# MaartenGr/PolyFuzz

Measured on AMD Instinct MI355X. Metric: string-pairs/sec, TF-IDF cosine top-n 100k x 100k (config.timed_step says what a step is: by default the user-level .match() call of SURVEY section 8d's metric, `device_step` = the list resident in HBM; latency.top1_single_query_ms = top-1 match latency), higher is better.
Workload: dtype f32

## Files before the change

include/polyfuzz_hip.h:

```cpp
#ifndef POLYFUZZ_HIP_H
#define POLYFUZZ_HIP_H

#include <stdint.h>

#ifdef __cplusplus
extern "C" {
#endif

#define PFZ_VERSION 100

typedef enum pfz_status {
    PFZ_OK = 0,
    PFZ_ERR_INVALID = -1,
    PFZ_ERR_NO_DEVICE = -2,
    PFZ_ERR_HIP = -3,
    PFZ_ERR_UNSUPPORTED = -4,
    PFZ_ERR_NOMEM = -5,
    PFZ_ERR_RCCL = -6
} pfz_status;

typedef struct pfz_ctx pfz_ctx;
typedef struct pfz_csr pfz_csr;
typedef struct pfz_index pfz_index;
typedef struct pfz_topn pfz_topn;
// ... 22 lines not shown

int pfz_csr_upload(pfz_ctx *ctx, int64_t n_rows, int64_t n_cols,
                   const int64_t *indptr, const int32_t *indices, const float *data,
                   pfz_csr **out);
int pfz_csr_shape(const pfz_csr *m, int64_t *n_rows, int64_t *n_cols, int64_t *nnz);
int pfz_csr_download(pfz_ctx *ctx, const pfz_csr *m, int64_t *indptr, int32_t *indices, float *data);
void pfz_csr_free(pfz_csr *m);

int pfz_index_build(pfz_ctx *ctx, const pfz_csr *to_matrix, pfz_index **out);
void pfz_index_free(pfz_index *ix);
int pfz_index_info(const pfz_index *ix, int64_t *n_rows, int64_t *n_cols, int64_t *nnz,
                   int64_t *block_cols, int64_t *n_blocks, int64_t *table_bytes);
int pfz_index_pieces(const pfz_index *ix, int64_t *n_pieces, int64_t *piece_postings);
int pfz_index_symmetric_launches(const pfz_index *ix, int64_t *launches, int64_t *rows);
int pfz_index_symmetric_census(const pfz_index *ix, int64_t *magnet_rows, int64_t *recomputed_rows);

int pfz_topn_alloc(pfz_ctx *ctx, int64_t n_rows, int32_t ntop, pfz_topn **out);
void pfz_topn_free(pfz_topn *t);
int pfz_topn_clear(pfz_ctx *ctx, pfz_topn *t);
int pfz_topn_download(pfz_ctx *ctx, const pfz_topn *t, int32_t *out_idx, float *out_val);
int pfz_topn_download_rows_after(pfz_ctx *ctx, const pfz_topn *t, int64_t row_begin, int64_t row_end,
                                 int32_t event_slot, int32_t *out_idx, float *out_val);
int pfz_topn_rows_begin(pfz_ctx *ctx, const pfz_topn *t, int64_t row_begin, int64_t row_end, int32_t event_slot, int32_t half);
int pfz_topn_rows_finish(pfz_ctx *ctx, int32_t half, const int32_t **idx, const float **val);
int pfz_topn_upload(pfz_ctx *ctx, pfz_topn *t, const int32_t *idx, const float *val);
int pfz_topn_device_ptrs(const pfz_topn *t, void **idx_dev, void **val_dev, int64_t *n_rows, int32_t *ntop);

int pfz_cossim_topn(pfz_ctx *ctx, const pfz_index *to_index, const pfz_csr *from_matrix,
                    int32_t ntop, float lower_bound, int32_t exclude_diag, int64_t diag_offset,
                    pfz_topn *out);
// ... 203 lines not shown
```

polyfuzz_amd/_lib.py:

```python
import ctypes
import os
import threading

import numpy as np

from . import _build

c_i32, c_i64, c_f32, c_f64 = ctypes.c_int32, ctypes.c_int64, ctypes.c_float, ctypes.c_double
c_vp = ctypes.c_void_p
P = ctypes.POINTER


class PfzError(RuntimeError):
    def __init__(self, code, msg):
        super().__init__(f"libpolyfuzz_hip error {code}: {msg}")
        self.code = code


class PfzUnsupported(PfzError, NotImplementedError):
    pass


class PfzNoDevice(PfzError):
    pass
# ... 16 lines not shown
    "pfz_event_record": (ctypes.c_int, [c_vp, c_i32]),
    "pfz_event_elapsed_ms": (ctypes.c_int, [c_vp, c_i32, c_i32, P(c_f32)]),
    "pfz_prof_enable": (ctypes.c_int, [c_vp, c_i32]),
    "pfz_prof_reset": (ctypes.c_int, [c_vp]),
    "pfz_prof_get": (ctypes.c_int, [c_vp, ctypes.c_char_p, P(c_f64), P(c_i64)]),
    "pfz_csr_upload": (ctypes.c_int, [c_vp, c_i64, c_i64, c_vp, c_vp, c_vp, P(c_vp)]),
    "pfz_csr_shape": (ctypes.c_int, [c_vp, P(c_i64), P(c_i64), P(c_i64)]),
    "pfz_csr_download": (ctypes.c_int, [c_vp, c_vp, c_vp, c_vp, c_vp]),
    "pfz_csr_free": (None, [c_vp]),
    "pfz_index_build": (ctypes.c_int, [c_vp, c_vp, P(c_vp)]),
    "pfz_index_free": (None, [c_vp]),
    "pfz_index_info": (ctypes.c_int, [c_vp, P(c_i64), P(c_i64), P(c_i64), P(c_i64), P(c_i64), P(c_i64)]),
    "pfz_index_pieces": (ctypes.c_int, [c_vp, P(c_i64), P(c_i64)]),
    "pfz_index_symmetric_launches": (ctypes.c_int, [c_vp, P(c_i64), P(c_i64)]),
    "pfz_index_symmetric_census": (ctypes.c_int, [c_vp, P(c_i64), P(c_i64)]),
    "pfz_index_symmetric_ok": (ctypes.c_int, [c_vp, c_vp, c_i32, c_i32, P(c_i32)]),
    "pfz_comm_cossim_topn_symmetric": (ctypes.c_int, [c_vp, c_vp, c_vp, c_i32, ctypes.c_float, c_vp]),
    "pfz_comm_symmetric_ok": (ctypes.c_int, [c_vp, c_vp, c_vp, c_i32, P(c_i32)]),
    "pfz_rccl_versions": (ctypes.c_int, [P(c_i32), P(c_i32)]),
    "pfz_topn_alloc": (ctypes.c_int, [c_vp, c_i64, c_i32, P(c_vp)]),
    "pfz_topn_free": (None, [c_vp]),
    "pfz_topn_download": (ctypes.c_int, [c_vp, c_vp, c_vp, c_vp]),
    "pfz_topn_clear": (ctypes.c_int, [c_vp, c_vp]),
    "pfz_topn_download_rows_after": (ctypes.c_int, [c_vp, c_vp, c_i64, c_i64, c_i32, c_vp, c_vp]),
    "pfz_topn_rows_begin": (ctypes.c_int, [c_vp, c_vp, c_i64, c_i64, c_i32, c_i32]),
    "pfz_topn_rows_finish": (ctypes.c_int, [c_vp, c_i32, P(c_vp), P(c_vp)]),
    "pfz_cossim_topn_ranges": (ctypes.c_int, [c_vp, c_vp, c_vp, c_i32, ctypes.c_float, c_i32, c_i32, P(c_i64), c_i32, c_vp, P(c_vp), P(c_vp)]),
    "pfz_event_wait": (ctypes.c_int, [c_vp, c_i32]),
    "pfz_stage_reserve": (ctypes.c_int, [c_vp, c_i64, P(c_vp)]),
    "pfz_topn_upload": (ctypes.c_int, [c_vp, c_vp, c_vp, c_vp]),
# ... 281 lines not shown
    def symmetric_launches(self):
        a, b = c_i64(), c_i64()
        check(self.ctx.lib.pfz_index_symmetric_launches(self.h, ctypes.byref(a), ctypes.byref(b)))
        return a.value, b.value

    def symmetric_ok(self, csr, ntop, n_parts=1):
        yes = c_i32()
        check(self.ctx.lib.pfz_index_symmetric_ok(self.h, csr.h, int(ntop), int(n_parts), ctypes.byref(yes)))
        return bool(yes.value)

    def symmetric_census(self):
        a, b = c_i64(), c_i64()
        check(self.ctx.lib.pfz_index_symmetric_census(self.h, ctypes.byref(a), ctypes.byref(b)))
        return a.value, b.value


class DeviceTopN(_Handle):
    _free = "pfz_topn_free"

    @classmethod
    def alloc(cls, ctx, n_rows, ntop):
        h = c_vp()
        check(ctx.lib.pfz_topn_alloc(ctx.h, int(n_rows), int(ntop), ctypes.byref(h)))
        t = cls(ctx, h)
        t.n_rows, t.ntop = int(n_rows), int(ntop)
        return t

    def download(self):
        idx = np.empty((self.n_rows, self.ntop), np.int32)
        val = np.empty((self.n_rows, self.ntop), np.float32)
# ... 1035 lines not shown
```

polyfuzz_amd/csrc/k3_symmetric.hip:

```cpp
#include "k3_core.h"

#include <stdio.h>
#include <stdlib.h>

namespace pfz {

constexpr int kSymC = 2048;
constexpr int kSymCap = 96;
constexpr int kSymKeep = 32;
#ifndef PFZ_K3_SYM_F
#define PFZ_K3_SYM_F 128
#endif
#ifndef PFZ_K3_SYM_PUSH
#define PFZ_K3_SYM_PUSH 512
#endif
constexpr int kSymF = PFZ_K3_SYM_F;
constexpr int kSymPush = PFZ_K3_SYM_PUSH;
constexpr int kSymMergeCap = kSymPush + 64;
#ifndef PFZ_K3_SYM_SIDE_STREAMS
#define PFZ_K3_SYM_SIDE_STREAMS 2
#endif
constexpr int kSymSides = PFZ_K3_SYM_SIDE_STREAMS;
static_assert(kSymSides >= 1 && kSymSides <= 4, "one to four side streams");
constexpr int kSymSlices = 8;
constexpr int kSymSlicedRows = 4096;
#ifndef PFZ_K3_SYM_EXP
#define PFZ_K3_SYM_EXP 0
#endif
constexpr int kSymMag = 1;
constexpr int kSymMagBlocks = 8;
constexpr int kSymP0PerCu = 128;
constexpr int kSymDoneStride = 32;
constexpr int kNoThr = 0x7fffffff;

struct K3SymArgs {
    const int32_t *a_indptr;
    const int32_t *a_idx;
    const float *a_val;
    int32_t n;
    const int32_t *tab;
    const int2 *post;
    const int2 *post_sym;
    const uint16_t *pblk;
    const int32_t *n_pieces1;
    int32_t nb, ntop, thr0;
    float scale, inv_scale;
    int32_t row_begin, row_end;
    int32_t n_parts, my_part, per;
    int32_t thr_by_part;
    uint64_t *keys_out;
    int32_t *thrv;
    uint16_t *slot4;
    uint32_t *gmin;
    int32_t *thr_slot;
    uint16_t *row_slot;
    int32_t *mag;
    int32_t n_mag_items, mag_b0, mag_row_end;
    uint64_t *keys;
    int32_t *push_cnt;
    uint64_t *push_buf;
    int32_t *ovf;
    uint64_t *part;
    int32_t ovf_base, ovf_max, n_sl;
    int32_t *out_idx;
    float *out_val;
    int32_t *host_idx;
    float *host_val;
    uint32_t *done;
    int32_t blk_lo, blk_hi;
};

// ... 1 lines not shown
{
    return a.thr_by_part ? (row % a.n_parts) * a.per + row / a.n_parts : row;
}
__device__ inline bool row_is_mine(const K3SymArgs &a, int row) { return a.n_parts == 1 || row % a.n_parts == a.my_part; }


__host__ __device__ inline int sym_slot(int rho, int i, int *t, int *l, int *e)
{
    const int p = i >> 1, half = i & 1, c = rho & 3;
    *t = p >> 3;
    *l = (rho >> 2) + 8 * (p & 7);
    *e = half * 4 + c;
    return 512 * *t + 256 * half + 4 * *l + c;
}

__global__ __launch_bounds__(1024) void k3_sym_order(const K3SymArgs a)
{
    __shared__ int s_gmin[256];
    const int b = blockIdx.x, lane = threadIdx.x & 63, wave = threadIdx.x >> 6;
    if (threadIdx.x < 256) s_gmin[threadIdx.x] = kNoThr;
    if (threadIdx.x == 0 && a.done) a.done[b * kSymDoneStride] = 0u;
    __syncthreads();
    for (int rho = wave * 2; rho < wave * 2 + 2; ++rho) {
        const int r = rho + 32 * lane;
        const int row = b * kSymC + r;
        if (row < a.n) a.push_cnt[row] = 0;
        const int thr = row < a.n ? a.thrv[thr_pos(a, row)] : kNoThr;
        const uint64_t key = ((uint64_t)(uint32_t)thr << 6) | (uint32_t)lane;
        int rank = 0;
#pragma unroll 16
        for (int m = 0; m < 64; ++m) {
            const uint32_t lo = (uint32_t)__builtin_amdgcn_readlane((int)(uint32_t)key, m);
            const uint32_t hi = (uint32_t)__builtin_amdgcn_readlane((int)(uint32_t)(key >> 32), m);
            rank += ((((uint64_t)hi << 32) | lo) < key) ? 1 : 0;
        }
        int t, l, e;
        const int slot = sym_slot(rho, rank, &t, &l, &e);
        const bool magnet = rank < kSymMag && row < a.n && b > 0;
        if (rank < kSymMag) a.mag[(int64_t)b * (32 * kSymMag) + rho * kSymMag + rank] = magnet ? row : -1;
        a.slot4[(int64_t)b * kSymC + r] = (uint16_t)(slot * 4);
        a.thr_slot[(int64_t)b * kSymC + slot] = magnet ? kNoThr : thr;
        a.row_slot[(int64_t)b * kSymC + slot] = (uint16_t)r;
        if (!magnet) atomicMin(&s_gmin[t * 64 + l], thr);
    }
    __syncthreads();
    if (threadIdx.x < 64) {
        uint32_t w = 0;
        for (int t = 0; t < 4; ++t) {
            const int g = s_gmin[t * 64 + threadIdx.x];
            w |= (g == kNoThr ? 0xffu : (uint32_t)g >> 24) << (8 * t);
        }
        a.gmin[(int64_t)b * 64 + threadIdx.x] = w;
    }
}

__global__ __launch_bounds__(256) void k3_sym_repost(const K3SymArgs a)
{
    const int64_t i = (int64_t)blockIdx.x * 256 + threadIdx.x;
    if (i >= (int64_t)*a.n_pieces1 * (kPiece / 2)) return;
    const int piece = (int)(i >> 3);
    const int b = a.pblk[piece];
    int4 e = ((const int4 *)a.post)[i];
    const uint16_t *s4 = a.slot4 + (int64_t)b * kSymC;
    if (piece > 0) {
        e.x = s4[e.x >> 2];
        e.z = s4[e.z >> 2];
    }
// ... 38 lines not shown
    }
    const uint64_t t0 = wall_clock64();
    for (int b0 = a.blk_lo; b0 < a.blk_hi; b0 += 64) {
        const int b = b0 + lane;
        const bool on = b < a.blk_hi;
        const uint32_t want = on ? sym_items_of_block(a, b) : 0u;
        for (;;) {
            const uint32_t got = on ? __hip_atomic_load(&a.done[b * kSymDoneStride], __ATOMIC_RELAXED, __HIP_MEMORY_SCOPE_AGENT) : 0u;
            if (!__ballot(got < want)) break;
            if (wall_clock64() - t0 > 1000000000ull) __builtin_trap();
            __builtin_amdgcn_s_sleep(32);
        }
    }
}

template <int kCap>
__device__ inline void drain_stage(uint64_t *cand, TopState &st, uint64_t *fbuf, int &fcnt, int ntop, int lane,
                                   const K3SymArgs &a, uint32_t inv_row)
{
    wave_sync();
    for (int e0 = 0; e0 < fcnt; e0 += 64) {
        const bool on = e0 + lane < fcnt;
        const uint64_t en = on ? fbuf[e0 + lane] : 0ull;
        const uint32_t lo = (uint32_t)en;
        const int cell = (int)(lo & 0x3fffffffu);
        const int x = (int)(uint32_t)(en >> 32);
        int rowl = 0, thr = kNoThr;
        if (on) {
            rowl = a.row_slot[cell];
            thr = a.thr_slot[cell];
        }
        const int row = (cell & ~(kSymC - 1)) + rowl;
#if PFZ_K3_SYM_EXP == 5
        if (false) {
#else
        if ((lo & kStageFgn) && x > thr) {
#endif
            const int pos = atomicAdd(&a.push_cnt[row], 1);
            if (pos < kSymPush) store_coherent(&a.push_buf[(int64_t)row * kSymPush + pos], (en & 0xffffffff00000000ull) | inv_row);
        }
        const bool own = (lo & kStageOwn) && x > st.thr;
        const uint64_t mo = __ballot(own);
        if (mo) {
            const int pos = st.cnt + __popcll(mo & ((1ull << lane) - 1ull));
            if (own) cand[pos] = (en & 0xffffffff00000000ull) | (uint32_t)(~row);
            st.cnt += __popcll(mo);
            st.pushed = 1;
            if (st.cnt > kCap - 64) compact<kCap>(cand, st, ntop, lane, false);
        }
    }
    wave_sync();
    fcnt = 0;
}

template <int kCap>
__device__ inline void stage1(uint64_t *cand, TopState &st, uint64_t *fbuf, int &fcnt, int x, uint32_t tgu, int cell, int ntop,
                              int lane, const K3SymArgs &a, uint32_t inv_row)
{
    const bool own = x > st.thr, fgn = (uint32_t)x >= tgu;
    const uint64_t mk = __ballot(own || fgn);
    if (mk) {
        const int pos = fcnt + __popcll(mk & ((1ull << lane) - 1ull));
        if (own || fgn)
            fbuf[pos] = ((uint64_t)(uint32_t)x << 32) | (own ? kStageOwn : 0u) | (fgn ? kStageFgn : 0u) | (uint32_t)cell;
        fcnt += __popcll(mk);
        if (fcnt > kSymF - 64) drain_stage<kCap>(cand, st, fbuf, fcnt, ntop, lane, a, inv_row);
    }
}

template <int kCap>
__device__ inline void stage8(uint64_t *cand, TopState &st, uint64_t *fbuf, int &fcnt, const int4 &v0, const int4 &v1, int pa,
                              int pb, int pc, uint32_t tgu, int cell0, int cell1, int ntop, int lane, const K3SymArgs &a,
                              uint32_t inv_row)
{
    if (__ballot(pa > st.thr || (uint32_t)pa >= tgu)) {
        stage1<kCap>(cand, st, fbuf, fcnt, v0.x, tgu, cell0, ntop, lane, a, inv_row);
        stage1<kCap>(cand, st, fbuf, fcnt, v0.y, tgu, cell0 + 1, ntop, lane, a, inv_row);
        stage1<kCap>(cand, st, fbuf, fcnt, v0.z, tgu, cell0 + 2, ntop, lane, a, inv_row);
    }
    if (__ballot(pb > st.thr || (uint32_t)pb >= tgu)) {
        stage1<kCap>(cand, st, fbuf, fcnt, v0.w, tgu, cell0 + 3, ntop, lane, a, inv_row);
        stage1<kCap>(cand, st, fbuf, fcnt, v1.x, tgu, cell1, ntop, lane, a, inv_row);
        stage1<kCap>(cand, st, fbuf, fcnt, v1.y, tgu, cell1 + 1, ntop, lane, a, inv_row);
    }
    if (__ballot(pc > st.thr || (uint32_t)pc >= tgu)) {
        stage1<kCap>(cand, st, fbuf, fcnt, v1.z, tgu, cell1 + 2, ntop, lane, a, inv_row);
        stage1<kCap>(cand, st, fbuf, fcnt, v1.w, tgu, cell1 + 3, ntop, lane, a, inv_row);
    }
}

template <int B> __device__ inline uint64_t top_byte_reaches(int mx, uint32_t q)
{
    uint64_t m;
    if (B == 0) asm("v_cmp_ge_u32_sdwa %0, %1, %2 src0_sel:BYTE_3 src1_sel:BYTE_0" : "=s"(m) : "v"(mx), "v"(q));
    else asm("v_cmp_ge_u32_sdwa %0, %1, %2 src0_sel:BYTE_3 src1_sel:BYTE_1" : "=s"(m) : "v"(mx), "v"(q));
    return m;
}

template <int N4, int kCap>
__device__ inline void sweep_block_handover(int4 *acc4, uint64_t *cand, TopState &st, int b, int ntop, int lane, int zero,
                                            uint32_t tq, uint64_t *fbuf, int &fcnt, const K3SymArgs &a, uint32_t inv_row)
{
    static_assert(N4 / 128 == 4, "four sweep steps per block");
#pragma unroll 1
    for (int h = 0; h < 2; ++h) {
#pragma unroll
        for (int u = 0; u < 2; ++u) {
            const int t = 2 * h + u;
            const int i0 = t * 128 + lane, i1 = i0 + 64;
            const int4 v0 = acc4[i0], v1 = acc4[i1];
            acc4[i0] = make_int4(zero, zero, zero, zero);
            acc4[i1] = make_int4(zero, zero, zero, zero);
            const int pa = max3i(v0.x, v0.y, v0.z), pb = max3i(v0.w, v1.x, v1.y), pc = max(v1.z, v1.w);
            const int mx = max3i(pa, pb, pc);
            const uint64_t hit = __ballot(mx > st.thr) | (u == 0 ? top_byte_reaches<0>(mx, tq) : top_byte_reaches<1>(mx, tq));
            if (hit)
                stage8<kCap>(cand, st, fbuf, fcnt, v0, v1, pa, pb, pc, (u == 0 ? tq << 24 : tq << 16) & 0xff000000u, b * kSymC + i0 * 4,
                             b * kSymC + i1 * 4, ntop, lane, a, inv_row);
        }
        tq >>= 16;
    }
}

__device__ inline void store_result(const K3SymArgs &a, int row, int r, uint64_t key)
{
    if (a.keys_out) {
        a.keys_out[(int64_t)row * a.ntop + r] = key;
    } else {
        const int32_t j = key ? (int32_t)(~(uint32_t)key) : -1;
        const float v = key ? (float)(int32_t)(uint32_t)(key >> 32) * a.inv_scale : 0.f;
        a.out_idx[(int64_t)row * a.ntop + r] = j;
        a.out_val[(int64_t)row * a.ntop + r] = v;
        if (a.host_idx) {
// ... 41 lines not shown
    const int n_sl = mode == 2 ? a.n_sl : 1;
    const int per_sl = (nb + n_sl - 1) / n_sl;
    if (mode == 2) {
        int n_ovf = a.ovf[0];
        n_ovf = n_ovf > a.n ? a.n : n_ovf;
        const int hi = n_ovf < a.ovf_base + a.ovf_max ? n_ovf : a.ovf_base + a.ovf_max;
        n_items = hi > a.ovf_base ? (hi - a.ovf_base) * n_sl : 0;
    }
    bool pf_ready = false;
    int pf_p0 = 0, pf_p1 = 0, pf_k = 0, pf_cur = 0, pf_nxt = 0;
    float pf_v = 0.f;
    for (int item = blockIdx.x; item < n_items; item += gridDim.x) {
        int row = mode == 2 ? a.ovf[1 + a.ovf_base + item / n_sl] : a.row_begin + item * a.n_parts;
        bool magnet = false;
        int m_lo = 0;
        if (mode == 1) {
            if (item < a.n_mag_items) {
                const int ns = (nb - 1 + kSymMagBlocks - 1) / kSymMagBlocks;
                const int mm = item / ns;
                m_lo = (item - mm * ns) * kSymMagBlocks;
                const int mblk = a.mag_b0 + mm / (32 * kSymMag);
                row = __builtin_amdgcn_readfirstlane(a.mag[(int64_t)mblk * (32 * kSymMag) + mm % (32 * kSymMag)]);
                if (row < a.row_begin || row >= a.mag_row_end || m_lo >= row / C || !row_is_mine(a, row)) {
                    sym_item_done(a, mblk, lane);
                    continue;
                }
                magnet = true;
            } else {
                row -= a.n_mag_items * a.n_parts;
                if (row >= (nb - 1) * C) continue;
            }
        }
        const int own = row / C;
        int b_lo = 0, b_hi = nb, b_first = own;
        if (mode == 2 && n_sl > 1) {
            b_lo = (item % n_sl) * per_sl;
            b_hi = b_lo + per_sl < nb ? b_lo + per_sl : nb;
            b_first = own >= b_lo && own < b_hi ? own : b_lo;
            if (b_lo >= b_hi) {
                if (lane < ntop) a.part[(int64_t)item * ntop + lane] = 0ull;
                continue;
            }
        }
        if (mode == 0) {
            b_lo = own;
// ... 11 lines not shown
            p0 = pf_p0;
            p1 = pf_p1;
        } else {
            p0 = a.a_indptr[row];
            p1 = a.a_indptr[row + 1];
        }
        const bool more = mode == 0 && item + (int)gridDim.x < n_items;
        const int row2 = a.row_begin + (item + (int)gridDim.x) * a.n_parts;
        int q0 = 0, q1 = 0;
        if (more) {
            q0 = a.a_indptr[row2];
            q1 = a.a_indptr[row2 + 1];
        }
        const int nnz = p1 - p0;
        const int self_col = mode == 1 ? -1 : row;
        const uint32_t inv_row = ~(uint32_t)row;
        TopState st;
        st.cnt = 0;
        st.thr = a.thr0;
        st.pushed = 0;
        bool warmed = false;
        if (mode == 1) {
            st.thr = a.thrv[thr_pos(a, row)];
            const uint64_t k = lane < ntop && !magnet ? a.keys[(int64_t)row * ntop + lane] : 0ull;
            st.cnt = __popcll(__ballot(k != 0ull));
            if (k) cand[lane] = k;
            warmed = true;
            wave_sync();
        }
        int fcnt = 0;

        const int n_blk = b_hi - b_lo;
        int cur0 = 0, nxt0 = 0;
        float as0 = 0.f;
        const bool have0 = lane < nnz;
        const int32_t *trow = a.tab;
        if (have0 && mode == 0 && pf_ready) {
            as0 = pf_v * a.scale;
            trow = a.tab + (int64_t)pf_k * nb;
            cur0 = pf_cur;
            nxt0 = pf_nxt;
        } else if (have0) {
            as0 = a.a_val[p0 + lane] * a.scale;
            trow = a.tab + (int64_t)a.a_idx[p0 + lane] * nb;
            cur0 = trow[b_first];
            nxt0 = trow[b_first + 1];
        }
        const bool have2 = more && lane < q1 - q0;

        uint32_t tq_next = 0xffffffffu;
#if PFZ_K3_SYM_EXP != 1
        if (mode == 1 && !magnet) tq_next = a.gmin[(int64_t)b_first * 64 + lane];
#endif
        for (int it = 0, b = b_first; it < n_blk; ++it) {
            const int s = cur0, e = have0 ? nxt0 : cur0;
            const int b_next = b + 1 < b_hi ? b + 1 : b_lo;
            const uint32_t tq = tq_next;
            bool touched = __ballot(e > s) != 0;
#if PFZ_K3_SYM_EXP == 13
            if (touched && mode != 0) scatter_pieces(acc, post_bytes, mark, e - s, s, as0, lane, src4, sub8, dummy_addr);
#else
// ... 24 lines not shown
                    scatter_pieces(acc, post_bytes, mark, e2 - s2, s2, as2, lane, src4, sub8, dummy_addr);
                }
            }
            if (touched) {
                wave_sync();
                if (!warmed) {
                    warmed = true;
#if PFZ_K3_SYM_EXP != 10
                    if (ntop <= kWarmMaxTop) {
                        const int t = warm_threshold<N4>(acc4, 0, ntop + 1, lane);
                        st.thr = t > st.thr ? t : st.thr;
                    }
#endif
                }
                if (mode == 1)
                    sweep_block_handover<N4, kSymCap>(acc4, cand, st, b, ntop, lane, zero, tq, fbuf, fcnt, a, inv_row);
#if PFZ_K3_SYM_EXP == 12
                else if (mode != 0)
#else
                else
#endif
                    sweep_block<N4, kSymCap>(acc4, cand, st, b * C, self_col, ntop, lane, zero);
                wave_sync();
            }
            if (mode == 0 && have2) {
                const int32_t *t2 = a.tab + (int64_t)pf_k * nb + row2 / C;
                pf_cur = t2[0];
                pf_nxt = t2[1];
            }
            b = b_next;
        }
        if (mode == 0) {
            pf_ready = more;
            pf_p0 = q0;
            pf_p1 = q1;
        }

        if (mode == 1 && fcnt) drain_stage<kSymCap>(cand, st, fbuf, fcnt, ntop, lane, a, inv_row);
#if PFZ_K3_SYM_EXP == 11
        if (mode != 0)
#endif
        compact<kSymCap>(cand, st, ntop, lane);
        if (mode == 1 && magnet) {
            if (lane < st.cnt) {
                const int pos = atomicAdd(&a.push_cnt[row], 1);
                if (pos < kSymPush) store_coherent(&a.push_buf[(int64_t)row * kSymPush + pos], cand[lane]);
            }
        } else if (mode == 2 && n_sl > 1) {
            if (lane < ntop) a.part[(int64_t)item * ntop + lane] = lane < st.cnt ? cand[lane] : 0ull;
        } else if (mode == 2) {
            for (int r = lane; r < ntop; r += 64) store_result(a, row, r, r < st.cnt ? cand[r] : 0ull);
        } else {
            if (lane < ntop) {
                const uint64_t k = lane < st.cnt ? cand[lane] : 0ull;
                if (mode == 1) store_coherent(&a.keys[(int64_t)row * ntop + lane], k);
                else a.keys[(int64_t)row * ntop + lane] = k;
            }
            if (mode == 0 && lane == 0) a.thrv[thr_pos(a, row)] = st.thr;
        }
        if (mode == 1) sym_item_done(a, own, lane);
        wave_sync();
// ... 64 lines not shown
            const uint64_t k = e0 + lane < total ? a.part[(int64_t)r * total + e0 + lane] : 0ull;
            const uint64_t mk = __ballot(k != 0ull);
            if (k) cand[st.cnt + __popcll(mk & ((1ull << lane) - 1ull))] = k;
            st.cnt += __popcll(mk);
        }
        compact<256>(cand, st, ntop, lane);
        for (int q = lane; q < ntop; q += 64) store_result(a, row, q, q < st.cnt ? cand[q] : 0ull);
        wave_sync();
    }
}


struct K3SymState {
    int64_t n = 0;
    DevBuf thrv, slot4, gmin, thr_slot, row_slot, mag, post_sym, keys, push_cnt, push_buf, ovf, part;
    DevBuf ovfx[3], partx[3];
    DevBuf done;
    int64_t next_row = -1;
    uint64_t a_serial = 0;
    const pfz_topn *out = nullptr;
    int32_t ntop = 0, thr0 = 0;
    float scale = 0.f;
    int64_t launches = 0, rows = 0;
};

void k3_sym_free(pfz_index *ix)
{
    delete ix->sym;
    ix->sym = nullptr;
}
// ... 16 lines not shown
    if (force == 1) return 1;
    if (ix->n_rows < knob_int(knob::K3_SYM_MIN, 20480) || ix->n_rows > 250000) return 0;
    return (row_end - row_begin) * 5 >= ix->n_rows ? 1 : 0;
}

static int sym_state_alloc(pfz_ctx *ctx, const pfz_index *ix, K3SymState *s)
{
    const int64_t n = ix->n_rows;
    const size_t cells = (size_t)ix->n_blocks * kSymC;
    PFZ_TRY(s->thrv.alloc(ctx, (size_t)(n + 64) * sizeof(int32_t)));
    PFZ_TRY(s->slot4.alloc(ctx, cells * sizeof(uint16_t)));
    PFZ_TRY(s->gmin.alloc(ctx, cells / 32 * sizeof(uint32_t)));
    PFZ_TRY(s->thr_slot.alloc(ctx, cells * sizeof(int32_t)));
    PFZ_TRY(s->row_slot.alloc(ctx, cells * sizeof(uint16_t)));
    PFZ_TRY(s->mag.alloc(ctx, (size_t)ix->n_blocks * 32 * kSymMag * sizeof(int32_t)));
    PFZ_TRY(s->post_sym.alloc(ctx, (size_t)ix->piece_cap * kPiece * sizeof(int2)));
    PFZ_TRY(s->keys.alloc(ctx, (size_t)n * kSymKeep * sizeof(uint64_t)));
    PFZ_TRY(s->push_cnt.alloc(ctx, (size_t)n * sizeof(int32_t)));
    PFZ_TRY(s->push_buf.alloc(ctx, (size_t)n * kSymPush * sizeof(uint64_t)));
    PFZ_TRY(s->ovf.alloc(ctx, (size_t)(n + 1) * sizeof(int32_t)));
    PFZ_TRY(s->part.alloc(ctx, (size_t)kSymSlicedRows * kSymSlices * kSymKeep * sizeof(uint64_t)));
    for (int q = 0; q + 1 < kSymSides; ++q) {
        PFZ_TRY(s->ovfx[q].alloc(ctx, (size_t)(n + 1) * sizeof(int32_t)));
        PFZ_TRY(s->partx[q].alloc(ctx, (size_t)kSymSlicedRows * kSymSlices * kSymKeep * sizeof(uint64_t)));
    }
    PFZ_TRY(s->done.alloc(ctx, (size_t)(ix->n_blocks + 64) * kSymDoneStride * sizeof(uint32_t)));
    return PFZ_OK;
}

static K3SymState *sym_state_of(pfz_ctx *ctx, const pfz_index *ix)
// ... 37 lines not shown
    a.scale = scale;
    a.inv_scale = inv_scale;
    a.row_begin = 0;
    a.row_end = (int32_t)ix->n_rows;
    a.n_parts = 1;
    a.my_part = 0;
    a.per = (int32_t)ix->n_rows;
    a.thr_by_part = 0;
    a.keys_out = nullptr;
    a.thrv = s->thrv.as<int32_t>();
    a.slot4 = s->slot4.as<uint16_t>();
    a.gmin = s->gmin.as<uint32_t>();
    a.thr_slot = s->thr_slot.as<int32_t>();
    a.row_slot = s->row_slot.as<uint16_t>();
    a.mag = s->mag.as<int32_t>();
    a.n_mag_items = 0;
    a.mag_b0 = 0;
    a.mag_row_end = 0;
    a.keys = s->keys.as<uint64_t>();
    a.push_cnt = s->push_cnt.as<int32_t>();
    a.push_buf = s->push_buf.as<uint64_t>();
    a.ovf = s->ovf.as<int32_t>();
    a.part = s->part.as<uint64_t>();
    a.ovf_base = 0;
    a.ovf_max = 0;
    a.n_sl = 1;
    a.out_idx = nullptr;
    a.out_val = nullptr;
    a.done = nullptr;
    a.blk_lo = a.blk_hi = 0;
// ... 238 lines not shown
    }
    float scale, inv_scale;
    int32_t thr0;
    k3_fixed_point(A, ix, lower_bound, &scale, &inv_scale, &thr0);
    s->next_row = -1;
    DevBuf mine, all;
    const size_t list_bytes = (size_t)n * ntop * sizeof(uint64_t);
    PFZ_TRY(mine.alloc(ctx, list_bytes));
    PFZ_TRY(all.alloc(ctx, list_bytes * n_parts));
    K3SymArgs a;
    sym_fill_args(a, ix, A, s, ntop, thr0, scale, inv_scale);
    a.n_parts = n_parts;
    a.my_part = part;
    a.per = (int32_t)((n + n_parts - 1) / n_parts);
    a.thr_by_part = 1;
    a.keys_out = mine.as<uint64_t>();
    PFZ_HIP(hipMemsetAsync(s->ovf.p, 0, sizeof(int32_t), ctx->stream));
    a.row_begin = part;
    a.row_end = (int32_t)n;
    const unsigned mine0 = (unsigned)((n - part + n_parts - 1) / n_parts);
    const unsigned grid0 = std::min<unsigned>(mine0, (unsigned)ctx->prop.multiProcessorCount * (unsigned)kSymP0PerCu);
    if (mine0) hipLaunchKernelGGL((k3_sym_kernel<kSymC, 0>), dim3(grid0), dim3(64), 0, ctx->stream, a);
    PFZ_HIP(hipGetLastError());
    if (n_parts > 1) PFZ_TRY(comm_allgather_bytes(comm, a.thrv + (size_t)part * a.per, a.thrv, (size_t)a.per * sizeof(int32_t)));
    hipLaunchKernelGGL(k3_sym_order, dim3((unsigned)nb), dim3(1024), 0, ctx->stream, a);
    const int64_t pairs = sym_repost_pairs(ix);
    hipLaunchKernelGGL(k3_sym_repost, dim3((unsigned)((pairs + 255) / 256)), dim3(256), 0, ctx->stream, a);
    const int64_t last_block_row = (int64_t)(nb - 1) * kSymC;
    a.row_end = (int32_t)(n < last_block_row ? n : last_block_row);
    const int rows1 = a.row_end > part ? (a.row_end - part + n_parts - 1) / n_parts : 0;
// ... 38 lines not shown
    const pfz::K3SymState *s = ix->sym;
    if (s && s->n > 0 && s->launches > 0) {
        PFZ_HIP(hipSetDevice(ix->ctx->device));
        std::vector<int32_t> mag((size_t)ix->n_blocks * 32 * pfz::kSymMag);
        int32_t n_ovf = 0;
        PFZ_TRY(pfz::copy_d2h(ix->ctx, mag.data(), s->mag.p, mag.size() * sizeof(int32_t)));
        PFZ_TRY(pfz::copy_d2h(ix->ctx, &n_ovf, s->ovf.p, sizeof(int32_t)));
        for (int32_t r : mag) mags += r >= 0;
        rec = n_ovf;
    }
    if (magnet_rows) *magnet_rows = mags;
    if (recomputed_rows) *recomputed_rows = rec;
    return PFZ_OK;
}

extern "C" int pfz_comm_cossim_topn_symmetric(pfz_comm *c, const pfz_index *ix, const pfz_csr *A, int32_t ntop, float lower_bound,
                                              pfz_topn *out)
{
    PFZ_REQUIRE(c && ix && A && out, "pfz_comm_cossim_topn_symmetric: NULL argument");
    PFZ_REQUIRE(ntop >= 1 && lower_bound == lower_bound, "pfz_comm_cossim_topn_symmetric: ntop must be >= 1 and lower_bound a number");
    PFZ_REQUIRE(out->n_rows >= A->n_rows && out->ntop == ntop, "pfz_comm_cossim_topn_symmetric: result buffer is %lldx%d, need %lldx%d",
                (long long)out->n_rows, out->ntop, (long long)A->n_rows, ntop);
    if (!pfz::k3_sym_sharded_ok(ix, A, ntop, pfz::comm_world(c))) {
        pfz::set_error("pfz_comm_cossim_topn_symmetric: not a job for the symmetric form (the matrix must be the one the index was built "
                       "from, 2048-row blocks, at least two of them, top_n <= 32, ranks x top_n <= 256): ask pfz_index_symmetric_ok first");
        return PFZ_ERR_UNSUPPORTED;
    }
    pfz_ctx *ctx = ix->ctx;
    PFZ_HIP(hipSetDevice(ctx->device));
    pfz::ProfScope ps(ctx, "k3_cossim_topn");
// ... 23 lines not shown
```

polyfuzz_amd/csrc/pfz_knobs.h:

```cpp
#pragma once

namespace pfz {

int knob_int(const char *name, int dflt);
bool knob_set(const char *name);
const char *knob_str(const char *name);

namespace knob {

inline constexpr const char *DEBUG_SYNC = "PFZ_DEBUG_SYNC";
inline constexpr const char *SCAN3 = "PFZ_SCAN3";
inline constexpr const char *K1_EXTRACT = "PFZ_K1_EXTRACT";
inline constexpr const char *K1_WAVE_STRINGS = "PFZ_K1_WAVE_STRINGS";
inline constexpr const char *K1_TWO_LISTS = "PFZ_K1_TWO_LISTS";
inline constexpr const char *K1_FUSE_ROWS = "PFZ_K1_FUSE_ROWS";
inline constexpr const char *NO_LDS_HIST = "PFZ_NO_LDS_HIST";
inline constexpr const char *K2_SELF_SCAN = "PFZ_K2_SELF_SCAN";
inline constexpr const char *K3_BLOCK = "PFZ_K3_BLOCK";
inline constexpr const char *K3_BANK_ORDER = "PFZ_K3_BANK_ORDER";
inline constexpr const char *K3_NO_BANK_ORDER = "PFZ_K3_NO_BANK_ORDER";
inline constexpr const char *K3_SLICES = "PFZ_K3_SLICES";
inline constexpr const char *K3_NO_STREAMED = "PFZ_K3_NO_STREAMED";
inline constexpr const char *K3_LOCKSTEP = "PFZ_K3_LOCKSTEP";
inline constexpr const char *K3_LS_MIN_TO = "PFZ_K3_LS_MIN_TO";
inline constexpr const char *K3_LS_BLOCKS = "PFZ_K3_LS_BLOCKS";
inline constexpr const char *K3_LS_WAVES = "PFZ_K3_LS_WAVES";
inline constexpr const char *K3_LS_CHUNK = "PFZ_K3_LS_CHUNK";
inline constexpr const char *K3_SYM = "PFZ_K3_SYM";
inline constexpr const char *K3_SYM_MIN = "PFZ_K3_SYM_MIN";
inline constexpr const char *K3_SYM_FAIL_ALLOC = "PFZ_K3_SYM_FAIL_ALLOC";
#ifdef PFZ_EXPERIMENTS
inline constexpr const char *K3_ABLATE = "PFZ_K3_ABLATE";
inline constexpr const char *K3_SYM_SOLO = "PFZ_K3_SYM_SOLO";
inline constexpr const char *K7_EXP = "PFZ_K7_EXP";
#endif
inline constexpr const char *K4_FORCE_GENERAL = "PFZ_K4_FORCE_GENERAL";
inline constexpr const char *K4_PARTS = "PFZ_K4_PARTS";
inline constexpr const char *K4_SIDE_STREAM = "PFZ_K4_SIDE_STREAM";
inline constexpr const char *K4_NO_QUAD = "PFZ_K4_NO_QUAD";
inline constexpr const char *K4_NO_OCTO = "PFZ_K4_NO_OCTO";
inline constexpr const char *K5_PANEL_ROWS = "PFZ_K5_PANEL_ROWS";
inline constexpr const char *K5_NO_OVERLAP = "PFZ_K5_NO_OVERLAP";
inline constexpr const char *K5_NO_BLOCK_MAX = "PFZ_K5_NO_BLOCK_MAX";
inline constexpr const char *K7_FORCE_GENERAL = "PFZ_K7_FORCE_GENERAL";
// ... 9 lines not shown
```

polyfuzz_amd/pipeline.py:

```python
import numpy as np

from . import _lib

PROFILED_KERNELS = ("k1_extract", "k2_rows_short", "k2_rows_long", "k2_df_hist", "k2_finalize", "k_index_count",
                    "k_index_fill", "k_index_bank_order", "k3_cossim_topn")


def shard_bounds(n, world, rank):
    base, rem = divmod(n, world)
    begin = rank * base + min(rank, rem)
    return begin, begin + base + (1 if rank < rem else 0)


def balanced_bounds(strings, world):
    n = len(strings)
    if world <= 1 or n == 0:
        return [(0, n)] + [(n, n)] * (max(world, 1) - 1)
    cost = np.fromiter((len(s) + 1 for s in strings), np.int64, n)
    cs = np.cumsum(cost)
    edges = [0] + [int(np.searchsorted(cs, cs[-1] * r // world, side="left")) for r in range(1, world)] + [n]
    edges = [min(max(e, 0), n) for e in edges]
    for i in range(1, len(edges)):
        edges[i] = max(edges[i], edges[i - 1])
    return list(zip(edges[:-1], edges[1:]))
# ... 131 lines not shown

    def stats(self):
        (fp, fi, _), (tp, ti, _), n_cols = self.host_matrices()
        df_from = np.bincount(fi, minlength=n_cols).astype(np.float64)
        df_to = np.bincount(ti, minlength=n_cols).astype(np.float64)
        out = {"vocab": int(n_cols), "nnz_from": int(fp[-1]), "nnz_to": int(tp[-1]),
               "madds": float((df_from * df_to).sum())}
        if self.from_csr is self.to_csr and self.index is not None:
            info = self.index.info()
            c, nb = info["block_cols"], info["n_blocks"]
            row_of = np.repeat(np.arange(len(tp) - 1, dtype=np.int64), np.diff(tp))
            per_list = np.bincount(ti.astype(np.int64) * nb + row_of // c, minlength=n_cols * nb).astype(np.float64)
            madds_diag = float((per_list * per_list).sum())
            out["madds_symmetric"] = 0.5 * (out["madds"] + madds_diag)
            out["cells_symmetric"] = float(((nb - np.arange(len(tp) - 1, dtype=np.int64) // c) * c).sum())
        return out


def sharded_self_match(ctx, comm, names, top_n=1, min_similarity=0.0, n_gram_range=(3, 3), clean_string=True,
                       remove_space_ngrams=True, engine=None):
    from .models._utils import topn_to_frame
    names = names if isinstance(names, list) else list(names)
    bounds = balanced_bounds(names, comm.world) if len(names) > 250_000 else [shard_bounds(len(names), comm.world, r) for r in range(comm.world)]
    b, e = bounds[comm.rank]
    sizes = [y - x for x, y in bounds]
    job = TfidfMatchJob(ctx, names[b:e], names, top_n=top_n, min_similarity=min_similarity, n_gram_range=n_gram_range,
                        clean_string=clean_string, remove_space_ngrams=remove_space_ngrams, comm=comm, self_match=True,
                        shard_offset=b, rows_per_rank=max(sizes), engine=engine)
    idx, val = job.step().download()
    idx, val = job.whole_result(idx, val, sizes)
    return topn_to_frame(np.ascontiguousarray(idx, np.int32), np.ascontiguousarray(val, np.float32), names, names, top_n)
# ... 191 lines not shown
```

Before: 3651 billion.

## Deduplicate identical rows per block in symmetric top-n, sweeping only class leaders

During the symmetric cosine top-n pass, the code hashes each row's TF-IDF vector and groups identical rows within a block into classes in the order kernel. Only the class leader sweeps the cross-block region; copies skip their sweep and receive the leader's candidates, and foreign pushes are fanned out to every member. This cuts redundant similarity work when the string list contains duplicates, at the cost of extra hashing, LDS class building, more buffers and more atomics. It is on by default and disabled for multi-part runs.

```diff
diff --git a/include/polyfuzz_hip.h b/include/polyfuzz_hip.h
--- a/include/polyfuzz_hip.h
+++ b/include/polyfuzz_hip.h
@@ -60,6 +60,7 @@
 int pfz_index_pieces(const pfz_index *ix, int64_t *n_pieces, int64_t *piece_postings);
 int pfz_index_symmetric_launches(const pfz_index *ix, int64_t *launches, int64_t *rows);
 int pfz_index_symmetric_census(const pfz_index *ix, int64_t *magnet_rows, int64_t *recomputed_rows);
+int pfz_index_symmetric_copies(const pfz_index *ix, int64_t *classes, int64_t *copies);
 
 int pfz_topn_alloc(pfz_ctx *ctx, int64_t n_rows, int32_t ntop, pfz_topn **out);
 void pfz_topn_free(pfz_topn *t);
diff --git a/polyfuzz_amd/_lib.py b/polyfuzz_amd/_lib.py
--- a/polyfuzz_amd/_lib.py
+++ b/polyfuzz_amd/_lib.py
@@ -54,6 +54,7 @@
     "pfz_index_pieces": (ctypes.c_int, [c_vp, P(c_i64), P(c_i64)]),
     "pfz_index_symmetric_launches": (ctypes.c_int, [c_vp, P(c_i64), P(c_i64)]),
     "pfz_index_symmetric_census": (ctypes.c_int, [c_vp, P(c_i64), P(c_i64)]),
+    "pfz_index_symmetric_copies": (ctypes.c_int, [c_vp, P(c_i64), P(c_i64)]),
     "pfz_index_symmetric_ok": (ctypes.c_int, [c_vp, c_vp, c_i32, c_i32, P(c_i32)]),
     "pfz_comm_cossim_topn_symmetric": (ctypes.c_int, [c_vp, c_vp, c_vp, c_i32, ctypes.c_float, c_vp]),
     "pfz_comm_symmetric_ok": (ctypes.c_int, [c_vp, c_vp, c_vp, c_i32, P(c_i32)]),
@@ -365,6 +366,11 @@
         check(self.ctx.lib.pfz_index_symmetric_census(self.h, ctypes.byref(a), ctypes.byref(b)))
         return a.value, b.value
 
+    def symmetric_copies(self):
+        a, b = c_i64(), c_i64()
+        check(self.ctx.lib.pfz_index_symmetric_copies(self.h, ctypes.byref(a), ctypes.byref(b)))
+        return a.value, b.value
+
 
 class DeviceTopN(_Handle):
     _free = "pfz_topn_free"
diff --git a/polyfuzz_amd/csrc/k3_symmetric.hip b/polyfuzz_amd/csrc/k3_symmetric.hip
--- a/polyfuzz_amd/csrc/k3_symmetric.hip
+++ b/polyfuzz_amd/csrc/k3_symmetric.hip
@@ -32,6 +32,7 @@
 constexpr int kSymP0PerCu = 128;
 constexpr int kSymDoneStride = 32;
 constexpr int kNoThr = 0x7fffffff;
+constexpr uint32_t kSymCopy = 0xffffffffu;
 
 struct K3SymArgs {
     const int32_t *a_indptr;
@@ -55,6 +56,11 @@
     int32_t *thr_slot;
     uint16_t *row_slot;
     int32_t *mag;
+    int32_t copies;
+    uint32_t *rhash;
+    uint32_t *cls;
+    uint16_t *memb;
+    int32_t *thr_cls;
     int32_t n_mag_items, mag_b0, mag_row_end;
     uint64_t *keys;
     int32_t *push_cnt;
@@ -86,18 +92,143 @@
     return 512 * *t + 256 * half + 4 * *l + c;
 }
 
+struct SymClassLds {
+    uint32_t tab[2 * kSymC];
+    uint32_t hash[kSymC];
+    uint32_t cls[kSymC];
+    int thr[kSymC];
+    uint16_t lead[kSymC];
+    int total;
+};
+
+__device__ inline bool sym_rows_equal(const K3SymArgs &a, int r0, int r1)
+{
+    const int p0 = a.a_indptr[r0], p1 = a.a_indptr[r1];
+    const int nnz = a.a_indptr[r0 + 1] - p0;
+    if (a.a_indptr[r1 + 1] - p1 != nnz) return false;
+    uint32_t diff = 0u;
+    for (int k0 = 0; k0 < nnz && !diff; k0 += 16) {
+#pragma unroll
+        for (int u = 0; u < 16; ++u) {
+            const int k = k0 + u < nnz ? k0 + u : nnz - 1;
+            diff |= (uint32_t)(a.a_idx[p0 + k] ^ a.a_idx[p1 + k]) | (__float_as_uint(a.a_val[p0 + k]) ^ __float_as_uint(a.a_val[p1 + k]));
+        }
+    }
+    return diff == 0u;
+}
+
+__device__ inline void sym_class_enter(const K3SymArgs &a, SymClassLds &s, int b, int r, int thr)
+{
+    const int row = b * kSymC + r;
+    s.hash[r] = row < a.n ? a.rhash[row] : 0u;
+    s.cls[r] = 0u;
+    s.thr[r] = thr;
+    s.lead[r] = (uint16_t)r;
+}
+
+__device__ inline void sym_classes(const K3SymArgs &a, SymClassLds &s, int b, int r0)
+{
+    constexpr uint32_t kMask = 2 * kSymC - 1;
+    int *const fill = (int *)s.tab;
+    uint16_t *const stage = (uint16_t *)(s.tab + kSymC);
+    int slot[2] = {0, 0};
+    for (int q = 0; q < 2; ++q) {
+        const int r = r0 + q;
+        const uint32_t h = s.hash[r];
+        if (!h) continue;
+        uint32_t at = h & kMask;
+        for (;;) {
+            const uint32_t old = atomicCAS(&s.tab[at], kSymCopy, (uint32_t)r);
+            if (old == kSymCopy) break;
+            if (s.hash[old] == h) {
+                atomicMin(&s.tab[at], (uint32_t)r);
+                break;
+            }
+            at = (at + 1) & kMask;
+        }
+        slot[q] = (int)at;
+    }
+    __syncthreads();
+    for (int q = 0; q < 2; ++q) {
+        const int r = r0 + q;
+        const uint32_t h = s.hash[r];
+        if (!h) continue;
+        const int first = (int)s.tab[slot[q]];
+        if (first == r) continue;
+        int lead = r;
+        if (sym_rows_equal(a, b * kSymC + r, b * kSymC + first)) {
+            lead = first;
+        } else {
+            for (int c = first + 1; c < r; ++c)
+                if (s.hash[c] == h && sym_rows_equal(a, b * kSymC + r, b * kSymC + c)) {
+                    lead = c;
+                    break;
+                }
+        }
+        if (lead != r) {
+            s.lead[r] = (uint16_t)lead;
+            atomicAdd(&s.cls[lead], 1u);
+            atomicMin(&s.thr[lead], s.thr[r]);
+        }
+    }
+    __syncthreads();
+    for (int q = 0; q < 2; ++q) {
+        const int r = r0 + q;
+        const uint32_t copies = s.cls[r];
+        if (!copies) continue;
+        const int off = atomicAdd(&s.total, (int)copies + 1);
+        s.cls[r] = ((uint32_t)off << 16) | (copies + 1u);
+        fill[r] = 0;
+        stage[off] = (uint16_t)r;
+    }
+    __syncthreads();
+    for (int q = 0; q < 2; ++q) {
+        const int r = r0 + q;
+        const int lead = s.lead[r];
+        if (lead == r) continue;
+        stage[(s.cls[lead] >> 16) + 1 + atomicAdd(&fill[lead], 1)] = (uint16_t)r;
+    }
+    __syncthreads();
+    for (int q = 0; q < 2; ++q) {
+        const int r = r0 + q;
+        const int64_t cell = (int64_t)b * kSymC + r;
+        const int lead = s.lead[r];
+        const uint32_t w = s.cls[lead];
+        const int off = (int)(w >> 16), members = (int)(w & 0xffffu);
+        if (lead != r) {
+            int rank = 0;
+            for (int k = 1; k < members; ++k) rank += stage[off + k] < r ? 1 : 0;
+            a.memb[(int64_t)b * kSymC + off + 1 + rank] = (uint16_t)r;
+        } else if (w) {
+            a.memb[(int64_t)b * kSymC + off] = (uint16_t)r;
+        }
+        a.cls[cell] = lead != r ? kSymCopy : w;
+        a.thr_cls[cell] = s.thr[r];
+    }
+    for (int i = threadIdx.x; i < kSymC; i += 1024)
+        if (i >= s.total) a.memb[(int64_t)b * kSymC + i] = 0;
+}
+
 __global__ __launch_bounds__(1024) void k3_sym_order(const K3SymArgs a)
 {
     __shared__ int s_gmin[256];
+    __shared__ SymClassLds s_cls;
     const int b = blockIdx.x, lane = threadIdx.x & 63, wave = threadIdx.x >> 6;
     if (threadIdx.x < 256) s_gmin[threadIdx.x] = kNoThr;
     if (threadIdx.x == 0 && a.done) a.done[b * kSymDoneStride] = 0u;
+    if (a.copies) {
+        for (int i = threadIdx.x; i < 2 * kSymC; i += 1024) s_cls.tab[i] = kSymCopy;
+        if (threadIdx.x == 0) s_cls.total = 0;
+    }
+    int thr2[2];
     __syncthreads();
     for (int rho = wave * 2; rho < wave * 2 + 2; ++rho) {
         const int r = rho + 32 * lane;
         const int row = b * kSymC + r;
         if (row < a.n) a.push_cnt[row] = 0;
         const int thr = row < a.n ? a.thrv[thr_pos(a, row)] : kNoThr;
+        thr2[rho & 1] = thr;
+        if (a.copies) sym_class_enter(a, s_cls, b, r, thr);
         const uint64_t key = ((uint64_t)(uint32_t)thr << 6) | (uint32_t)lane;
         int rank = 0;
 #pragma unroll 16
@@ -123,6 +254,16 @@
             w |= (g == kNoThr ? 0xffu : (uint32_t)g >> 24) << (8 * t);
         }
         a.gmin[(int64_t)b * 64 + threadIdx.x] = w;
+    }
+    if (a.copies) {
+        sym_classes(a, s_cls, b, wave * 2 + 32 * lane);
+    } else {
+        for (int q = 0; q < 2; ++q) {
+            const int64_t cell = (int64_t)b * kSymC + wave * 2 + q + 32 * lane;
+            a.cls[cell] = 0u;
+            a.memb[cell] = 0;
+            a.thr_cls[cell] = thr2[q];
+        }
     }
 }
 
@@ -191,9 +332,14 @@
     }
 }
 
+struct SymFrom {
+    uint32_t inv_row;
+    uint32_t cls;
+};
+
 template <int kCap>
 __device__ inline void drain_stage(uint64_t *cand, TopState &st, uint64_t *fbuf, int &fcnt, int ntop, int lane,
-                                   const K3SymArgs &a, uint32_t inv_row)
+                                   const K3SymArgs &a, const SymFrom &from)
 {
     wave_sync();
     for (int e0 = 0; e0 < fcnt; e0 += 64) {
@@ -213,8 +359,18 @@
 #else
         if ((lo & kStageFgn) && x > thr) {
 #endif
-            const int pos = atomicAdd(&a.push_cnt[row], 1);
-            if (pos < kSymPush) store_coherent(&a.push_buf[(int64_t)row * kSymPush + pos], (en & 0xffffffff00000000ull) | inv_row);
+            if (from.cls == 0u) {
+                const int pos = atomicAdd(&a.push_cnt[row], 1);
+                if (pos < kSymPush) store_coherent(&a.push_buf[(int64_t)row * kSymPush + pos], (en & 0xffffffff00000000ull) | from.inv_row);
+            } else {
+                const uint32_t blk_row = ~from.inv_row & ~(uint32_t)(kSymC - 1);
+                const int members = (int)(from.cls & 0xffffu), memb_at = (int)(blk_row + (from.cls >> 16));
+                for (int m = 0; m < members; ++m) {
+                    const uint32_t inv = ~(blk_row + a.memb[memb_at + m]);
+                    const int pos = atomicAdd(&a.push_cnt[row], 1);
+                    if (pos < kSymPush) store_coherent(&a.push_buf[(int64_t)row * kSymPush + pos], (en & 0xffffffff00000000ull) | inv);
+                }
+            }
         }
         const bool own = (lo & kStageOwn) && x > st.thr;
         const uint64_t mo = __ballot(own);
@@ -232,7 +388,7 @@
 
 template <int kCap>
 __device__ inline void stage1(uint64_t *cand, TopState &st, uint64_t *fbuf, int &fcnt, int x, uint32_t tgu, int cell, int ntop,
-                              int lane, const K3SymArgs &a, uint32_t inv_row)
+                              int lane, const K3SymArgs &a, const SymFrom &from)
 {
     const bool own = x > st.thr, fgn = (uint32_t)x >= tgu;
     const uint64_t mk = __ballot(own || fgn);
@@ -241,28 +397,28 @@
         if (own || fgn)
             fbuf[pos] = ((uint64_t)(uint32_t)x << 32) | (own ? kStageOwn : 0u) | (fgn ? kStageFgn : 0u) | (uint32_t)cell;
         fcnt += __popcll(mk);
-        if (fcnt > kSymF - 64) drain_stage<kCap>(cand, st, fbuf, fcnt, ntop, lane, a, inv_row);
+        if (fcnt > kSymF - 64) drain_stage<kCap>(cand, st, fbuf, fcnt, ntop, lane, a, from);
     }
 }
 
 template <int kCap>
 __device__ inline void stage8(uint64_t *cand, TopState &st, uint64_t *fbuf, int &fcnt, const int4 &v0, const int4 &v1, int pa,
                               int pb, int pc, uint32_t tgu, int cell0, int cell1, int ntop, int lane, const K3SymArgs &a,
-                              uint32_t inv_row)
+                              const SymFrom &from)
 {
     if (__ballot(pa > st.thr || (uint32_t)pa >= tgu)) {
-        stage1<kCap>(cand, st, fbuf, fcnt, v0.x, tgu, cell0, ntop, lane, a, inv_row);
-        stage1<kCap>(cand, st, fbuf, fcnt, v0.y, tgu, cell0 + 1, ntop, lane, a, inv_row);
-        stage1<kCap>(cand, st, fbuf, fcnt, v0.z, tgu, cell0 + 2, ntop, lane, a, inv_row);
+        stage1<kCap>(cand, st, fbuf, fcnt, v0.x, tgu, cell0, ntop, lane, a, from);
+        stage1<kCap>(cand, st, fbuf, fcnt, v0.y, tgu, cell0 + 1, ntop, lane, a, from);
+        stage1<kCap>(cand, st, fbuf, fcnt, v0.z, tgu, cell0 + 2, ntop, lane, a, from);
     }
     if (__ballot(pb > st.thr || (uint32_t)pb >= tgu)) {
-        stage1<kCap>(cand, st, fbuf, fcnt, v0.w, tgu, cell0 + 3, ntop, lane, a, inv_row);
-        stage1<kCap>(cand, st, fbuf, fcnt, v1.x, tgu, cell1, ntop, lane, a, inv_row);
-        stage1<kCap>(cand, st, fbuf, fcnt, v1.y, tgu, cell1 + 1, ntop, lane, a, inv_row);
+        stage1<kCap>(cand, st, fbuf, fcnt, v0.w, tgu, cell0 + 3, ntop, lane, a, from);
+        stage1<kCap>(cand, st, fbuf, fcnt, v1.x, tgu, cell1, ntop, lane, a, from);
+        stage1<kCap>(cand, st, fbuf, fcnt, v1.y, tgu, cell1 + 1, ntop, lane, a, from);
     }
     if (__ballot(pc > st.thr || (uint32_t)pc >= tgu)) {
-        stage1<kCap>(cand, st, fbuf, fcnt, v1.z, tgu, cell1 + 2, ntop, lane, a, inv_row);
-        stage1<kCap>(cand, st, fbuf, fcnt, v1.w, tgu, cell1 + 3, ntop, lane, a, inv_row);
+        stage1<kCap>(cand, st, fbuf, fcnt, v1.z, tgu, cell1 + 2, ntop, lane, a, from);
+        stage1<kCap>(cand, st, fbuf, fcnt, v1.w, tgu, cell1 + 3, ntop, lane, a, from);
     }
 }
 
@@ -276,7 +432,7 @@
 
 template <int N4, int kCap>
 __device__ inline void sweep_block_handover(int4 *acc4, uint64_t *cand, TopState &st, int b, int ntop, int lane, int zero,
-                                            uint32_t tq, uint64_t *fbuf, int &fcnt, const K3SymArgs &a, uint32_t inv_row)
+                                            uint32_t tq, uint64_t *fbuf, int &fcnt, const K3SymArgs &a, const SymFrom &from)
 {
     static_assert(N4 / 128 == 4, "four sweep steps per block");
 #pragma unroll 1
@@ -293,7 +449,7 @@
             const uint64_t hit = __ballot(mx > st.thr) | (u == 0 ? top_byte_reaches<0>(mx, tq) : top_byte_reaches<1>(mx, tq));
             if (hit)
                 stage8<kCap>(cand, st, fbuf, fcnt, v0, v1, pa, pb, pc, (u == 0 ? tq << 24 : tq << 16) & 0xff000000u, b * kSymC + i0 * 4,
-                             b * kSymC + i1 * 4, ntop, lane, a, inv_row);
+                             b * kSymC + i1 * 4, ntop, lane, a, from);
         }
         tq >>= 16;
     }
@@ -365,6 +521,7 @@
         int row = mode == 2 ? a.ovf[1 + a.ovf_base + item / n_sl] : a.row_begin + item * a.n_parts;
         bool magnet = false;
         int m_lo = 0;
+        uint32_t cls_v = 0u;
         if (mode == 1) {
             if (item < a.n_mag_items) {
                 const int ns = (nb - 1 + kSymMagBlocks - 1) / kSymMagBlocks;
@@ -380,6 +537,7 @@
             } else {
                 row -= a.n_mag_items * a.n_parts;
                 if (row >= (nb - 1) * C) continue;
+                cls_v = a.cls[row];
             }
         }
         const int own = row / C;
@@ -421,7 +579,10 @@
         }
         const int nnz = p1 - p0;
         const int self_col = mode == 1 ? -1 : row;
-        const uint32_t inv_row = ~(uint32_t)row;
+        SymFrom from;
+        from.inv_row = ~(uint32_t)row;
+        from.cls = 0u;
+        bool leader = false;
         TopState st;
         st.cnt = 0;
         st.thr = a.thr0;
@@ -429,7 +590,18 @@
         bool warmed = false;
         if (mode == 1) {
             st.thr = a.thrv[thr_pos(a, row)];
-            const uint64_t k = lane < ntop && !magnet ? a.keys[(int64_t)row * ntop + lane] : 0ull;
+            uint64_t k = lane < ntop && !magnet ? a.keys[(int64_t)row * ntop + lane] : 0ull;
+            const uint32_t cls = (uint32_t)__builtin_amdgcn_readfirstlane((int)cls_v);
+            if (cls == kSymCopy) {
+                sym_item_done(a, own, lane);
+                continue;
+            }
+            if (cls != 0u) {
+                leader = true;
+                from.cls = cls;
+                st.thr = a.thr_cls[row];
+                k = 0ull;
+            }
             st.cnt = __popcll(__ballot(k != 0ull));
             if (k) cand[lane] = k;
             warmed = true;
@@ -442,16 +614,33 @@
         float as0 = 0.f;
         const bool have0 = lane < nnz;
         const int32_t *trow = a.tab;
+        int k0 = 0;
+        float v0 = 0.f;
         if (have0 && mode == 0 && pf_ready) {
-            as0 = pf_v * a.scale;
-            trow = a.tab + (int64_t)pf_k * nb;
+            k0 = pf_k;
+            v0 = pf_v;
+            as0 = v0 * a.scale;
+            trow = a.tab + (int64_t)k0 * nb;
             cur0 = pf_cur;
             nxt0 = pf_nxt;
         } else if (have0) {
-            as0 = a.a_val[p0 + lane] * a.scale;
-            trow = a.tab + (int64_t)a.a_idx[p0 + lane] * nb;
+            k0 = a.a_idx[p0 + lane];
+            v0 = a.a_val[p0 + lane];
+            as0 = v0 * a.scale;
+            trow = a.tab + (int64_t)k0 * nb;
             cur0 = trow[b_first];
             nxt0 = trow[b_first + 1];
+        }
+        if (mode == 0 && a.copies) {
+            uint32_t hv = 0u;
+            if (have0) {
+                hv = ((uint32_t)k0 ^ ((uint32_t)lane << 24)) * 0x85ebca6bu;
+                hv = (hv ^ (hv >> 13) ^ __float_as_uint(v0)) * 0xc2b2ae35u;
+                hv ^= hv >> 16;
+            }
+#pragma unroll
+            for (int m = 32; m >= 1; m >>= 1) hv += (uint32_t)__shfl_xor((int)hv, m, 64);
+            if (lane == 0) a.rhash[row] = nnz > 0 ? (hv + (uint32_t)nnz * 0x9e3779b1u) | 1u : 0u;
         }
         const bool have2 = more && lane < q1 - q0;
 
@@ -506,7 +695,7 @@
 #endif
                 }
                 if (mode == 1)
-                    sweep_block_handover<N4, kSymCap>(acc4, cand, st, b, ntop, lane, zero, tq, fbuf, fcnt, a, inv_row);
+                    sweep_block_handover<N4, kSymCap>(acc4, cand, st, b, ntop, lane, zero, tq, fbuf, fcnt, a, from);
 #if PFZ_K3_SYM_EXP == 12
                 else if (mode != 0)
 #else
@@ -528,7 +717,7 @@
             pf_p1 = q1;
         }
 
-        if (mode == 1 && fcnt) drain_stage<kSymCap>(cand, st, fbuf, fcnt, ntop, lane, a, inv_row);
+        if (mode == 1 && fcnt) drain_stage<kSymCap>(cand, st, fbuf, fcnt, ntop, lane, a, from);
 #if PFZ_K3_SYM_EXP == 11
         if (mode != 0)
 #endif
@@ -537,6 +726,14 @@
             if (lane < st.cnt) {
                 const int pos = atomicAdd(&a.push_cnt[row], 1);
                 if (pos < kSymPush) store_coherent(&a.push_buf[(int64_t)row * kSymPush + pos], cand[lane]);
+            }
+        } else if (mode == 1 && leader) {
+            const int members = (int)(from.cls & 0xffffu), memb_at = own * C + (int)(from.cls >> 16);
+            for (int m = lane; m < members && st.cnt > 0; m += 64) {
+                const int mrow = own * C + a.memb[memb_at + m];
+                const int pos = atomicAdd(&a.push_cnt[mrow], st.cnt);
+                for (int k = 0; k < st.cnt; ++k)
+                    if (pos + k < kSymPush) store_coherent(&a.push_buf[(int64_t)mrow * kSymPush + pos + k], cand[k]);
             }
         } else if (mode == 2 && n_sl > 1) {
             if (lane < ntop) a.part[(int64_t)item * ntop + lane] = lane < st.cnt ? cand[lane] : 0ull;
@@ -631,6 +828,7 @@
 struct K3SymState {
     int64_t n = 0;
     DevBuf thrv, slot4, gmin, thr_slot, row_slot, mag, post_sym, keys, push_cnt, push_buf, ovf, part;
+    DevBuf rhash, cls, memb, thr_cls;
     DevBuf ovfx[3], partx[3];
     DevBuf done;
     int64_t next_row = -1;
@@ -677,6 +875,10 @@
     PFZ_TRY(s->thr_slot.alloc(ctx, cells * sizeof(int32_t)));
     PFZ_TRY(s->row_slot.alloc(ctx, cells * sizeof(uint16_t)));
     PFZ_TRY(s->mag.alloc(ctx, (size_t)ix->n_blocks * 32 * kSymMag * sizeof(int32_t)));
+    PFZ_TRY(s->rhash.alloc(ctx, cells * sizeof(uint32_t)));
+    PFZ_TRY(s->cls.alloc(ctx, cells * sizeof(uint32_t)));
+    PFZ_TRY(s->memb.alloc(ctx, cells * sizeof(uint16_t)));
+    PFZ_TRY(s->thr_cls.alloc(ctx, cells * sizeof(int32_t)));
     PFZ_TRY(s->post_sym.alloc(ctx, (size_t)ix->piece_cap * kPiece * sizeof(int2)));
     PFZ_TRY(s->keys.alloc(ctx, (size_t)n * kSymKeep * sizeof(uint64_t)));
     PFZ_TRY(s->push_cnt.alloc(ctx, (size_t)n * sizeof(int32_t)));
@@ -744,6 +946,11 @@
     a.thr_slot = s->thr_slot.as<int32_t>();
     a.row_slot = s->row_slot.as<uint16_t>();
     a.mag = s->mag.as<int32_t>();
+    a.copies = knob_int(knob::K3_SYM_COPIES, 1) != 0 ? 1 : 0;
+    a.rhash = s->rhash.as<uint32_t>();
+    a.cls = s->cls.as<uint32_t>();
+    a.memb = s->memb.as<uint16_t>();
+    a.thr_cls = s->thr_cls.as<int32_t>();
     a.n_mag_items = 0;
     a.mag_b0 = 0;
     a.mag_row_end = 0;
@@ -1012,6 +1219,7 @@
     a.my_part = part;
     a.per = (int32_t)((n + n_parts - 1) / n_parts);
     a.thr_by_part = 1;
+    a.copies = n_parts == 1 ? a.copies : 0;
     a.keys_out = mine.as<uint64_t>();
     PFZ_HIP(hipMemsetAsync(s->ovf.p, 0, sizeof(int32_t), ctx->stream));
     a.row_begin = part;
@@ -1080,6 +1288,25 @@
     return PFZ_OK;
 }
 
+extern "C" int pfz_index_symmetric_copies(const pfz_index *ix, int64_t *classes, int64_t *copies)
+{
+    PFZ_REQUIRE(ix, "pfz_index_symmetric_copies: NULL index");
+    int64_t n_cls = 0, n_cop = 0;
+    const pfz::K3SymState *s = ix->sym;
+    if (s && s->n > 0 && s->launches > 0) {
+        PFZ_HIP(hipSetDevice(ix->ctx->device));
+        std::vector<uint32_t> cls((size_t)ix->n_rows);
+        PFZ_TRY(pfz::copy_d2h(ix->ctx, cls.data(), s->cls.p, cls.size() * sizeof(uint32_t)));
+        for (uint32_t w : cls) {
+            n_cop += w == pfz::kSymCopy;
+            n_cls += w != 0u && w != pfz::kSymCopy;
+        }
+    }
+    if (classes) *classes = n_cls;
+    if (copies) *copies = n_cop;
+    return PFZ_OK;
+}
+
 extern "C" int pfz_comm_cossim_topn_symmetric(pfz_comm *c, const pfz_index *ix, const pfz_csr *A, int32_t ntop, float lower_bound,
                                               pfz_topn *out)
 {
diff --git a/polyfuzz_amd/csrc/pfz_knobs.h b/polyfuzz_amd/csrc/pfz_knobs.h
--- a/polyfuzz_amd/csrc/pfz_knobs.h
+++ b/polyfuzz_amd/csrc/pfz_knobs.h
@@ -28,6 +28,7 @@
 inline constexpr const char *K3_LS_CHUNK = "PFZ_K3_LS_CHUNK";
 inline constexpr const char *K3_SYM = "PFZ_K3_SYM";
 inline constexpr const char *K3_SYM_MIN = "PFZ_K3_SYM_MIN";
+inline constexpr const char *K3_SYM_COPIES = "PFZ_K3_SYM_COPIES";
 inline constexpr const char *K3_SYM_FAIL_ALLOC = "PFZ_K3_SYM_FAIL_ALLOC";
 #ifdef PFZ_EXPERIMENTS
 inline constexpr const char *K3_ABLATE = "PFZ_K3_ABLATE";
diff --git a/polyfuzz_amd/pipeline.py b/polyfuzz_amd/pipeline.py
--- a/polyfuzz_amd/pipeline.py
+++ b/polyfuzz_amd/pipeline.py
@@ -169,7 +169,28 @@
             madds_diag = float((per_list * per_list).sum())
             out["madds_symmetric"] = 0.5 * (out["madds"] + madds_diag)
             out["cells_symmetric"] = float(((nb - np.arange(len(tp) - 1, dtype=np.int64) // c) * c).sum())
+            if self.index.symmetric_copies()[1] > 0:
+                tv = self.to_csr.download()[2]
+                copies = copy_rows(tp, ti, tv, c)
+                above = per_list.reshape(n_cols, nb)[:, ::-1].cumsum(axis=1)[:, ::-1] - per_list.reshape(n_cols, nb)
+                for r in copies:
+                    out["madds_symmetric"] -= float(above[ti[tp[r]:tp[r + 1]], r // c].sum())
+                    out["cells_symmetric"] -= float((nb - 1 - r // c) * c)
+                out["rows_copies"] = len(copies)
         return out
+
+
+def copy_rows(indptr, indices, data, block):
+    data = np.ascontiguousarray(data, np.float32).view(np.uint32)
+    seen, copies = set(), []
+    for r in range(len(indptr) - 1):
+        a, b = int(indptr[r]), int(indptr[r + 1])
+        if b > a:
+            key = (r // block, indices[a:b].tobytes(), data[a:b].tobytes())
+            if key in seen:
+                copies.append(r)
+            seen.add(key)
+    return copies
 
 
 def sharded_self_match(ctx, comm, names, top_n=1, min_similarity=0.0, n_gram_range=(3, 3), clean_string=True,
```

Result: faster. 3715 billion, median of 6 (+1.8%).
